# Gabriel-Ducrocq/GibbsSampler

Measured on AMD Instinct MI355X. Metric: Gibbs iters/sec (constrained-realization + C_l draw), Nside=512 lmax=1024, higher is better.
Workload: dtype f64

## Files before the change

gibbssampler_amd/_capi.py:

```python
import contextlib
import ctypes
import os

_HERE = os.path.dirname(os.path.abspath(__file__))
LIB_PATH = os.environ.get("GIBBS_HIP_LIB", os.path.join(_HERE, "libgibbs_hip.so"))

GS_MODE_CENTERED = 0
GS_MODE_NONCENTERED = 1
GS_QUIRK_ASIS_RECENTRE_CENTERED = 1
GS_NPARAM = 10
GS_ALM_REAL = 0
GS_ALM_COMPLEX = 1
GS_MCR_AUX, GS_MCR_OVERRELAX, GS_MCR_MALA, GS_MCR_AUX_MALA = 0, 1, 2, 3
NSTAT = {1: 2, 2: 4, 3: 8}

c_int_p = ctypes.POINTER(ctypes.c_int)
c_double_p = ctypes.POINTER(ctypes.c_double)


class GsModelDesc(ctypes.Structure):
    _fields_ = [
        ("lmax", ctypes.c_int),
        ("nside", ctypes.c_int),
        ("nfields", ctypes.c_int),
# ... 24 lines not shown
        ("mu_eps", ctypes.c_double),
        ("adj_iter", ctypes.c_int),
        ("nchains", ctypes.c_int),
        ("sht_mode", ctypes.c_int),
    ]


class GibbsHipError(RuntimeError):
    pass


_lib = None

_VP = ctypes.c_void_p
_SIGS = [
    ("gs_abi_version", ctypes.c_int, []),
    ("gs_last_error", ctypes.c_char_p, []),
    ("gs_option_set", ctypes.c_int, [ctypes.c_char_p, ctypes.c_char_p]),
    ("gs_option_get", ctypes.c_char_p, [ctypes.c_char_p]),
    ("gs_plan_create", ctypes.c_int, [ctypes.POINTER(GsModelDesc), ctypes.POINTER(_VP)]),
    ("gs_plan_destroy", ctypes.c_int, [_VP]),
    ("gs_plan_info", ctypes.c_int, [_VP, c_int_p, c_int_p, c_int_p, c_int_p]),
    ("gs_plan_sweep_info", ctypes.c_int, [_VP, c_int_p, c_int_p]),
    ("gs_var_expand", ctypes.c_int, [ctypes.c_int, ctypes.c_int, _VP, _VP, _VP]),
    ("gs_real_to_complex", ctypes.c_int, [ctypes.c_int, ctypes.c_int, _VP, _VP, _VP]),
    ("gs_complex_to_real", ctypes.c_int, [ctypes.c_int, ctypes.c_int, _VP, _VP, _VP]),
    ("gs_remove_monopole_dipole", ctypes.c_int, [ctypes.c_int, ctypes.c_int, _VP, _VP]),
    ("gs_alm2cl", ctypes.c_int, [ctypes.c_int, ctypes.c_int, _VP, _VP, _VP, _VP]),
    ("gs_unfold_bins", ctypes.c_int, [ctypes.c_int, _VP, _VP, ctypes.c_int, _VP, _VP]),
    ("gs_block_params", ctypes.c_int, [_VP, ctypes.c_int, _VP, _VP, _VP]),
    ("gs_cr_sweep", ctypes.c_int, [_VP, _VP, _VP, _VP, ctypes.c_uint64, ctypes.c_uint32, ctypes.c_uint32,
                                   _VP, _VP, _VP]),
    ("gs_sweep_stats", ctypes.c_int, [_VP, _VP, _VP, _VP, _VP]),
    ("gs_cls_draw", ctypes.c_int, [_VP, _VP, _VP, ctypes.c_uint64, ctypes.c_uint32, _VP, _VP]),
    ("gs_cls_scale_trace", ctypes.c_int, [_VP, _VP, ctypes.c_int, _VP]),
    ("gs_nc_mh", ctypes.c_int, [_VP, _VP, _VP, _VP, _VP, ctypes.c_uint64, ctypes.c_uint32, _VP, _VP]),
    ("gs_mh_adapt_enable", ctypes.c_int, [_VP, ctypes.c_double, ctypes.c_double]),
    ("gs_mh_adapt", ctypes.c_int, [_VP, _VP, _VP]),
    ("gs_mh_scale_get", ctypes.c_int, [_VP, _VP, _VP, _VP]),
    ("gs_mh_scale_set", ctypes.c_int, [_VP, _VP, _VP, _VP]),
    ("gs_mh_proposal_sd", ctypes.c_int, [_VP, _VP, _VP]),
    ("gs_stats_to_noncentered", ctypes.c_int, [_VP, _VP, _VP, _VP]),
    ("gs_recentre", ctypes.c_int, [_VP, _VP, _VP, _VP, _VP]),
    ("gs_step_centered", ctypes.c_int, [_VP, _VP, _VP, _VP, _VP, _VP, ctypes.c_uint64, ctypes.c_uint32, _VP]),
    ("gs_step_asis_fused", ctypes.c_int, [_VP, _VP, _VP, _VP, ctypes.c_uint64, ctypes.c_uint32, _VP, _VP, ctypes.c_int,
                                          _VP, ctypes.c_int, _VP]),
# ... 197 lines not shown
```

gibbssampler_amd/build.py:

```python
import glob
import os
import subprocess
import sys

HERE = os.path.dirname(os.path.abspath(__file__))
ROOT = os.path.dirname(HERE)
SOURCES = [os.path.join(HERE, "csrc", "gs_kernels.hip"), os.path.join(HERE, "csrc", "gs_sht.hip"),
           os.path.join(HERE, "csrc", "gs_masked.hip"), os.path.join(HERE, "csrc", "gs_summary.hip"),
           os.path.join(HERE, "csrc", "gs_br.hip")]
HEADERS = [os.path.join(HERE, "csrc", h) for h in ("gs_rng.h", "gs_common.h", "gs_bm_tables.h", "gs_block.h",
                                                         "gs_launch.h")] + \
    [os.path.join(ROOT, "include", "gibbs_capi.h")]
LIB = os.path.join(HERE, "libgibbs_hip.so")
ARCH = os.environ.get("GIBBS_OFFLOAD_ARCH", "gfx950")
COMMON = ["-ffp-contract=on"]
VARIANTS = {
    None: (LIB, ["-O3"] + COMMON),
    "debug": (os.path.join(HERE, "libgibbs_hip_debug.so"), ["-O3", "-DGS_DEBUG"] + COMMON),
    "timeline": (os.path.join(HERE, "libgibbs_hip_timeline.so"), ["-O3", "-DGS_MH_TIMELINE"] + COMMON),
    "asan": (os.path.join(HERE, "libgibbs_hip_asan.so"),
             ["-O1", "-g", "-fno-omit-frame-pointer", "-Xarch_host", "-fsanitize=address", "-shared-libasan"] + COMMON),
}


def asan_runtime():
    hits = sorted(glob.glob("/opt/rocm/lib/llvm/lib/clang/*/lib/linux/libclang_rt.asan-x86_64.so"))
    return hits[-1] if hits else None


def _stale(target, deps):
    if not os.path.exists(target):
        return True
    t = os.path.getmtime(target)
    return any(os.path.getmtime(d) > t for d in deps)
# ... 33 lines not shown
```

gibbssampler_amd/csrc/gs_kernels.hip:

```cpp
#include <hip/hip_runtime.h>
#include <stdint.h>
#include <math.h>
#include <string>
#include <vector>
#include <cstring>
#include <algorithm>
#include <cstdlib>
#include <map>
#include <mutex>

#include "gibbs_capi.h"
#include "gs_rng.h"
#include "gs_common.h"
#include "gs_block.h"
#include "gs_launch.h"

using namespace gs;

namespace {

using gs_detail::set_error;
using gs_detail::with_F;
using gs_detail::SeedWords;
using gs_detail::seed_words;
using gs_detail::nblk;

constexpr int WAVE = 64;
constexpr int NP = GS_NPARAM;
constexpr double PI = 3.14159265358979323846;

inline int nstat_of(int F) { return F == 1 ? GS_NSTAT_1 : (F == 2 ? GS_NSTAT_2 : GS_NSTAT_3); }
inline int nspec_of(int F) { return F == 1 ? 1 : (F == 2 ? 2 : 4); }

}

struct gs_plan {
    int device = 0;
    int L = 0, nside = 0, Npix = 0, F = 0, nchains = 0, chain0 = 0, quirks = 0, n_iter_mh = 1;
// ... 23 lines not shown
    int phase_sp[4][2] = {{-1, -1}, {-1, -1}, {-1, -1}, {-1, -1}};
    int* ell2blk = nullptr;
    double* gbuf = nullptr;
    double* bl = nullptr;
    int* ell2bin = nullptr;
    int* bins = nullptr;
    int* blocks = nullptr;
    double* prop_sd = nullptr;
    bool adapt_on = false;
    double adapt_target = 0.25, adapt_kappa = 0.6, adapt_lmax = 20.0;
    int nblk_mh = 0;
    std::vector<int> bin2blk_h;
    int* bin2blk = nullptr;
    double* mh_lam = nullptr;
    int* mh_cnt = nullptr;
    double* sd_chain = nullptr;
    int sd_stride = 0;
    const double* sd_tab() const { return adapt_on ? sd_chain : prop_sd; }
    int* meta = nullptr;
    int2* tasks = nullptr;
    int npair = 0, ntile = 0, nchunk = 0, rows_per_task = 64;
    int sweep_tw = 4, nchunkg = 0;
    int ntask = 0;
    double* partials = nullptr;
    bool raw_on = true;
    double* dmom = nullptr;
    const double* dmom_src = nullptr;
    double* params = nullptr;
    double* stats = nullptr;
    double* prop = nullptr;
    double* logr = nullptr;
    double* dl_tmp = nullptr;
    double* u_nat = nullptr;
    uint32_t* iter_dev = nullptr;
    bool cls_pre = false;
    bool cls_pre_many = false;
    double* cls_var = nullptr;
    double* scale_tr = nullptr;
    int scale_cap = 1;
    struct Deferred {
        bool pro_pending = false;
        const double* pro_dl = nullptr;
        gs_detail::SeedWords pro_seed{0, 0};
        uint32_t pro_it = 0;
        bool u_nat_ready = false;
        bool snap_ok = false;
// ... 407 lines not shown
    int n = 0;
    int nbp = 0, nbu = 0;
    int nspec = 0, nacc = 0, n_iter_mh = 0, maxbins = 0;
    const int* nbins = nullptr;
    const double* prop_sd = nullptr;
    int sd_stride = 0;
    const double* dl = nullptr;
    double* prop = nullptr;
    double* logr = nullptr;
    double* u_out = nullptr;
    double* snap = nullptr;
    int nbv = 0;
    ClsPre cp{};
};
template <int F>
__device__ void pro_pre_item(const ProPre& pp, int bx, int nchains, uint32_t seed_lo, uint32_t seed_hi, IterArg itarg,
                             int chain0);

#if defined(GS_SWEEP_WGTIME)
constexpr int SW_TL_MAX = 16384;
__device__ unsigned long long g_sw_tl[4 * SW_TL_MAX];
#endif

template <int F, int ZM, bool STORE, bool RAW = false>
__device__ __forceinline__ void cr_sweep_task(int wg, int L, int nchains, int ntile, int nchunkg, int tm, int tw,
                                              const int2* __restrict__ tasks, const double* __restrict__ d,
                                              const double* __restrict__ params, const double* __restrict__ z,
                                              double* __restrict__ s, double* __restrict__ partials,
                                              uint32_t seed_lo, uint32_t seed_hi, uint32_t iter, uint32_t substep,
                                              int chain0, const SweepOp& op, const double* __restrict__ tab,
                                              double* red) {
    constexpr int NS = SweepAcc<F>::n(RAW);
    const int pair = wg / nchains;
    const int chain = wg % nchains;
    const int lane = threadIdx.x & 63;
    const int2 gc = tasks[pair];
    if (gc.x < 0) return;
    const int w = threadIdx.x >> 6, cw = 4 / tw;
    const int t = tw * gc.x + w % tw;
    const bool tile_ok = t < ntile;
    const int lhi = L - WAVE * t;
    const int m0 = (cw * gc.y + w / tw) * tm;
    const int m1 = min(m0 + tm, lhi + 1);
    const bool active = tile_ok && m0 < m1;
    GS_ASSERT(gc.y < nchunkg && gc.x * tw < ntile);
    const int ell_lo = lhi - 63;
    const int ell = ell_lo + lane;
    const bool lane_ok = ell >= 0;
    const long long NR = (long long)(L + 1) * (L + 1);
    const Key key = chain_key(seed_lo, seed_hi, (uint32_t)(chain0 + chain));
    const uint32_t tag = TAG_CR | (substep << 8);

    double pm[NP];
    sweep_operator<F>(ZM != 2 && (!RAW || STORE) && lane_ok && active, chain, ell, L, params, op, pm);
    double acc[NS];
#pragma unroll
    for (int q = 0; q < NS; ++q) acc[q] = 0.0;

    const double* zc = ZM == 1 ? z + (long long)chain * F * NR : nullptr;
    double* sc = s + (long long)chain * F * NR;
// ... 43 lines not shown
                sweep_entry<F, ZM, STORE, 2, RAW>(dv, zc, sc, NR, (long long)r, i32, tag, iter, key, pm, acc, tab);
            }
            i32 += (uint32_t)(L - m);
        }
    } else {
        for (; m < m1; ++m) {
            if (lane_ok && ell >= m) {
                load_d<F, 2>(d, NR, 2 * i - (L + 1), dv);
                sweep_entry<F, ZM, STORE, 2, RAW>(dv, zc, sc, NR, 2 * i - (L + 1), (uint32_t)i, tag, iter, key, pm,
                                                 acc, tab);
            }
            i += L - m;
        }
    }
    double* po = partials + (((long long)chain * ntile + t) * nchunkg + gc.y) * NS * WAVE;
    sweep_partials_store<NS>(acc, tw, w, lane, tile_ok && (cw * gc.y) * tm <= lhi, po, red);
}

#ifndef GS_SWEEP_MINW
#define GS_SWEEP_MINW 1
#endif
template <int F, int ZM, bool STORE, int PRE = 0, bool RAW = false>
__global__ __launch_bounds__(256, GS_SWEEP_MINW) void k_cr_sweep(int L, int nchains, int ntile, int nchunkg, int tm, int tw,
                                                  const int2* __restrict__ tasks, const double* __restrict__ d,
                                                  const double* __restrict__ params, const double* __restrict__ z,
                                                  double* __restrict__ s, double* __restrict__ partials,
                                                  uint32_t seed_lo, uint32_t seed_hi, IterArg itarg, uint32_t substep,
                                                  int chain0, SweepOp op, ClsPre cp, ProPre pp, int nlog) {
    if constexpr (PRE == 0 && ZM == 0) {
        if ((int)blockIdx.x < pp.n) {
            pro_pre_item<F>(pp, (int)blockIdx.x, nchains, seed_lo, seed_hi, itarg, chain0);
            return;
        }
    }
    const uint32_t iter = itarg.get();
    constexpr int NS = SweepAcc<F>::n(RAW);
    __shared__ __attribute__((aligned(16))) double tab[ZM == 0 ? BM_TAB_DOUBLES : 2];
    __shared__ double red[3 * NS * WAVE];
    if constexpr (PRE > 0) {
        static_assert(ZM == 0, "latency form: native draws only");
        const int nsw = (int)gridDim.x - cp.n;
        if ((int)blockIdx.x >= nsw) {
            cls_variates_item<F>(cp, ((int)blockIdx.x - nsw) * blockDim.x + threadIdx.x, seed_lo, seed_hi, iter,
                                 chain0);
            return;
        }
        cr_sweep_latency<F, STORE, PRE, RAW>(L, nchains, ntile, nchunkg, tm, tw, tasks, d, s, partials, seed_lo,
                                        seed_hi, iter, substep, chain0, op, tab, red, (int)blockIdx.x, nsw);
        return;
    }
    if constexpr (ZM == 0) {
        bm_stage_tables(tab);
        __syncthreads();
    }
    const int bid = (int)blockIdx.x - pp.n;
    const int xcd = bid & 7, q8 = nlog >> 3, r8 = nlog & 7;
    const int base = xcd < r8 ? xcd * (q8 + 1) : r8 * (q8 + 1) + (xcd - r8) * q8;
#if defined(GS_SWEEP_WGTIME)
    const unsigned long long tl0 = wall_clock64();
#endif
    cr_sweep_task<F, ZM, STORE, RAW>(base + (bid >> 3), L, nchains, ntile, nchunkg, tm, tw, tasks, d, params, z, s,
                                partials, seed_lo, seed_hi, iter, substep, chain0, op, tab, red);
#if defined(GS_SWEEP_WGTIME)
    __syncthreads();
    if (threadIdx.x == 0 && bid < SW_TL_MAX) {
        unsigned long long* o = g_sw_tl + 4 * (size_t)bid;
        o[0] = tl0;
        o[1] = wall_clock64();
        o[2] = __builtin_amdgcn_s_getreg((31 << 11) | 4);
        o[3] = __builtin_amdgcn_s_getreg((31 << 11) | 20);
    }
#endif
}

template <int G>
__device__ __forceinline__ double stats_finish_sum(int L, int ntile, int nchunkg, int tm, int nstat,
                                                   const double* partials, int chain, int q, int t,
                                                   int w, int lane) {
    const int cmax = (L - WAVE * t) / tm;
    GS_ASSERT(cmax < nchunkg);
    const double* pp = partials + ((long long)chain * ntile + t) * nchunkg * nstat * WAVE + q * WAVE + lane;
    const long long cs = (long long)nstat * WAVE;
    double acc = 0.0;
    if constexpr (G <= 4) {
        int c = w;
// ... 1315 lines not shown
            const double r11 = An.a11 * t11;
            const double rB = An.aB * tB;
            for (int c = 0; c < nv; ++c) {
                const double sT = sc[0 * NR + r + c], sE = sc[1 * NR + r + c];
                sc[0 * NR + r + c] = r00 * sT;
                sc[1 * NR + r + c] = r10 * sT + r11 * sE;
                sc[2 * NR + r + c] *= rB;
            }
        }
    }
}

__global__ void k_iter_advance(uint32_t* it) { *it += 1u; }

__global__ void k_record_trace(long long n, const double* __restrict__ dl, double* __restrict__ trace, int capacity,
                               IterArg itarg) {
    const uint32_t it = itarg.get();
    const long long slot = (long long)((it + capacity - 1u) % (uint32_t)capacity);
    for (long long k = blockIdx.x * (long long)blockDim.x + threadIdx.x; k < n; k += (long long)gridDim.x * blockDim.x)
        trace[slot * n + k] = dl[k];
}

static const char* const k_options[] = {
    "GS_SWEEP_TW", "GS_SWEEP_THROUGHPUT", "GS_NC_RAW", "GS_NC_PIPE", "GS_MH_SPLIT", "GS_CLS_PRE", "GS_CLS_PRE_MANY", "GS_F2_GROUP_BYTES",
    "GS_F2_BATCH_BYTES", "GS_SHT_LDS_FFT_MAX", "GS_SHT_SEG", "GS_SHT_SYN", "GS_SHT_ANA", "GS_SHT_MERGE_RINGS",
    "GS_SHT_CONST_RINGS", "GS_SHT_BLOCKS_MFMA", "GS_SHT_BLK_STAGE", "GS_SHT_FUSED_AUX", "GS_SHT_MFMA_MAX_GB",
    "GS_SHT_RING_TW2"};
static bool opt_known(const char* name) {
    for (const char* k : k_options)
        if (std::strcmp(k, name) == 0) return true;
    return false;
}
static std::mutex& opt_mu() { static std::mutex m; return m; }
static std::map<std::string, std::string>& opt_tab() { static std::map<std::string, std::string> t; return t; }

const char* gs_detail::option(const char* name) {
    std::lock_guard<std::mutex> g(opt_mu());
    const auto it = opt_tab().find(name);
    return it == opt_tab().end() ? nullptr : it->second.c_str();
}

namespace {

template <typename T>
int dev_upload(T** dst, const std::vector<T>& src) {
    if (src.empty()) { *dst = nullptr; return 0; }
    GS_CHECK(hipMalloc((void**)dst, src.size() * sizeof(T)));
    GS_CHECK(hipMemcpy(*dst, src.data(), src.size() * sizeof(T), hipMemcpyHostToDevice));
    return 0;
}

template <typename T>
int dev_alloc(T** dst, size_t n) {
    GS_CHECK(hipMalloc((void**)dst, std::max<size_t>(n, 1) * sizeof(T)));
    GS_CHECK(hipMemset(*dst, 0, std::max<size_t>(n, 1) * sizeof(T)));
    return 0;
}

inline hipStream_t S(void* s) { return (hipStream_t)s; }

void build_tasks(gs_plan* p) {
    const int L = p->L;
    p->ntile = (L + 1 + WAVE - 1) / WAVE;
    auto waves = [&](int tm) {
        long long n = 0;
        for (int t = 0; t < p->ntile; ++t) n += (L - WAVE * t) / tm + 1;
        return n;
    };
    const int tm = L > 512 ? 16 : (L > 256 ? 4 : 8);
    p->rows_per_task = tm;
    p->nchunk = L / tm + 1;
    p->ntask = (int)waves(tm);
    int tw = 1;
    if (const char* env = gs_detail::option("GS_SWEEP_TW")) {
        const int v = atoi(env);
        if (v == 1 || v == 2 || v == 4) tw = v;
    }
    const int cw = 4 / tw;
    p->sweep_tw = tw;
    p->nchunkg = (p->nchunk + cw - 1) / cw;
    std::vector<std::pair<long long, int2>> work;
    for (int g = 0; tw * g < p->ntile; ++g)
        for (int c = 0; c * cw * tm <= L - WAVE * tw * g; ++c) {
            long long wl = 0;
            for (int t = tw * g; t < std::min(tw * g + tw, p->ntile); ++t) {
                const int lhi = L - WAVE * t, lo = std::max(lhi - 63, 0);
                for (int m = c * cw * tm; m < std::min((c + 1) * cw * tm, lhi + 1); ++m)
                    wl += lhi - std::max(lo, m) + 1;
            }
            work.push_back({wl, make_int2(g, c)});
        }
    std::stable_sort(work.begin(), work.end(), [](const auto& a, const auto& b) { return a.first > b.first; });
    const int per = (int)((work.size() + 7) / 8);
    std::vector<std::vector<int2>> bucket(8);
    std::vector<long long> load(8, 0);
    for (const auto& w : work) {
        int best = -1;
        for (int x = 0; x < 8; ++x)
            if ((int)bucket[x].size() < per && (best < 0 || load[x] < load[best])) best = x;
        bucket[best].push_back(w.second);
        load[best] += w.first;
    }
    std::vector<int2> tasks;
    for (int x = 0; x < 8; ++x) {
        for (const int2& t : bucket[x]) tasks.push_back(t);
        for (int k = (int)bucket[x].size(); k < per; ++k) tasks.push_back(make_int2(-1, 0));
    }
    p->npair = (int)tasks.size();
    dev_upload(&p->tasks, tasks);
}

int check_plan(const gs_plan* p) {
    if (!p) return set_error("null plan");
    return 0;
}

template <typename Fn>
void with_G(const gs_plan* p, Fn&& fn) {
    if (p->nchains <= 4) fn(std::integral_constant<int, 16>{});
    else fn(std::integral_constant<int, 4>{});
}

using SweepKernel = void (*)(int, int, int, int, int, int, const int2*, const double*, const double*, const double*,
                             double*, double*, uint32_t, uint32_t, IterArg, uint32_t, int, SweepOp, ClsPre, ProPre, int);

template <int F>
SweepKernel sweep_variant(bool lat, bool given, bool rep, bool raw, bool st) {
    if (lat && raw) return st ? k_cr_sweep<F, 0, true, 4, true> : k_cr_sweep<F, 0, false, 4, true>;
    if (lat) return st ? k_cr_sweep<F, 0, true, 4> : k_cr_sweep<F, 0, false, 4>;
    if (given) return k_cr_sweep<F, 2, false>;
    if (rep) return st ? k_cr_sweep<F, 1, true> : k_cr_sweep<F, 1, false>;
    if (raw) return st ? k_cr_sweep<F, 0, true, 0, true> : k_cr_sweep<F, 0, false, 0, true>;
    return st ? k_cr_sweep<F, 0, true> : k_cr_sweep<F, 0, false>;
}

}

extern "C" {

int gs_abi_version(void) { return GS_ABI_VERSION; }
const char* gs_last_error(void) { return gs_detail::g_last_error.c_str(); }

int gs_option_set(const char* name, const char* value) {
    if (!name || !opt_known(name)) return set_error(std::string("gs_option_set: unknown option ") + (name ? name : "(null)"));
    std::lock_guard<std::mutex> g(opt_mu());
    if (value) opt_tab()[name] = value; else opt_tab().erase(name);
// ... 174 lines not shown
    rc |= dev_alloc(&p->params, nc * (L + 1) * NP);
    rc |= dev_alloc(&p->stats, nc * p->nstat * (L + 1));
    rc |= dev_alloc(&p->prop, nc * p->nspec * maxbins);
    rc |= dev_alloc(&p->logr, nc * p->nspec * maxbins);
    rc |= dev_alloc(&p->dl_tmp, nc * p->nspec * maxbins);
    rc |= dev_alloc(&p->u_nat, nc * std::max(p->nacc, 1));
    rc |= dev_alloc(&p->iter_dev, 4);
    {
        const char* e = gs_detail::option("GS_CLS_PRE");
        p->cls_pre = e ? std::atoi(e) != 0 : p->nchains <= 4;
    }
    {
        const char* e = gs_detail::option("GS_CLS_PRE_MANY");
        p->cls_pre_many = !p->cls_pre && (e ? std::atoi(e) != 0 : true);
    }
    if (p->cls_pre || p->cls_pre_many) rc |= dev_alloc(&p->cls_var, nc * p->nspec * maxbins * 3);
    if (rc) { gs_plan_destroy(p); return -1; }
    *out = p;
    return 0;
}

int gs_plan_destroy(gs_plan* p) {
    if (!p) return 0;
    void* bufs[] = {p->iter_dev, p->ell2blk, p->gbuf, p->phase_tab, p->phase_rng, p->meta, p->bl, p->ell2bin, p->bins, p->blocks, p->prop_sd, p->tasks, p->partials, p->u_nat,
                    p->params, p->stats, p->prop, p->logr, p->dl_tmp, p->cls_var, p->phase_tab_s, p->phase_rng_s, p->dmom,
                    p->bin2blk, p->mh_lam, p->mh_cnt, p->sd_chain};
    for (void* b : bufs)
        if (b) (void)hipFree(b);
    if (p->pipe.slot[1]) (void)hipFree(p->pipe.slot[1]);
    for (hipEvent_t e : {p->pipe.ev_fork, p->pipe.ev_sweep[0], p->pipe.ev_sweep[1], p->pipe.ev_finish[0],
                         p->pipe.ev_finish[1]})
        if (e) (void)hipEventDestroy(e);
    if (p->pipe.side) (void)hipStreamDestroy(p->pipe.side);
    for (hipEvent_t e : p->ev) (void)hipEventDestroy(e);
    delete p;
    return 0;
}

int gs_plan_info(const gs_plan* p, int* maxbins, int* nstat, int* nblocks_total, int* nspec) {
    if (check_plan(p)) return -1;
    if (maxbins) *maxbins = p->maxbins;
    if (nstat) *nstat = p->nstat;
    if (nblocks_total) *nblocks_total = p->nacc;
    if (nspec) *nspec = p->nspec;
    return 0;
}

int gs_plan_sweep_info(const gs_plan* p, int* ntask, int* rows_per_task) {
    if (check_plan(p)) return -1;
    if (ntask) *ntask = p->ntask;
    if (rows_per_task) *rows_per_task = p->rows_per_task;
    return 0;
}

static int check_lmax_n(const char* fn, int lmax, int n, const void* a, const void* b) {
    if (lmax < 0 || n < 0) return set_error(std::string(fn) + ": lmax / n out of range");
    if (n > 0 && (!a || !b)) return set_error(std::string(fn) + ": null argument");
    return 0;
}

int gs_var_expand(int lmax, int n, const double* dl, double* var, void* stream) {
    if (check_lmax_n("gs_var_expand", lmax, n, dl, var)) return -1;
    if (n == 0) return 0;
    const long long nc = (long long)(lmax + 1) * (lmax + 2) / 2 * n;
    hipLaunchKernelGGL(k_var_expand, dim3(nblk(nc, 256)), dim3(256), 0, S(stream), lmax, n, dl, var);
    GS_LAUNCH_CHECK("k_var_expand");
    return 0;
}

int gs_real_to_complex(int lmax, int n, const double* re, double* cx, void* stream) {
    if (check_lmax_n("gs_real_to_complex", lmax, n, re, cx)) return -1;
    if (n == 0) return 0;
    const long long nc = (long long)(lmax + 1) * (lmax + 2) / 2 * n;
    hipLaunchKernelGGL(k_real_to_complex, dim3(nblk(nc, 256)), dim3(256), 0, S(stream), lmax, n, re, cx);
// ... 173 lines not shown
    bool raw = false;
    bool finish = true;
    SeedWords seed{0, 0};
    uint32_t iteration = 0, substep = 0;
    bool* cls_pre_done = nullptr;
    int slot = -1;
};

static int sweep_launch(gs_plan* p, const SweepReq& r, void* stream) {
    if (check_plan(p)) return -1;
    const bool raw_nost = r.raw && !r.s_out;
    if (!r.d_alm || !r.stats || (!r.given && !r.params && r.op_mode < 0 && !raw_nost) || (r.given && !r.s_out) ||
        ((r.op_mode >= 0 || r.raw) && !r.dl) || (r.raw && (r.given || r.z)))
        return set_error("gs_cr_sweep: null argument");
    const bool ahead = r.slot >= 0;
    if (ahead && (r.slot > 1 || !p->pipe.ready || !raw_nost || r.finish || r.cls_pre_done))
        return set_error("gs_cr_sweep: a sweep ahead is a raw-moment sweep alone, into a prepared slot");
    double* const partials = ahead ? p->pipe.slot[r.slot] : p->partials;
    if (!ahead) {
        p->defer.raw_pending = r.raw;
        p->defer.raw_dl = r.raw ? r.dl : nullptr;
    }
    const SweepOp op{r.op_mode, p->maxbins, r.dl, p->ell2bin, p->bl, p->kappa[0], p->kappa[1], p->kappa[2]};
    const int nlog = (int)((long long)p->nchains * p->npair);
    dim3 g((unsigned)nlog), b(256);
    hipEvent_t e0 = nullptr, e1 = nullptr;
    if (timing_begin(p, S(stream), &e0, &e1)) return -1;
    const bool rep = r.z != nullptr, st = r.s_out != nullptr;
    const bool lat = r.op_mode >= 0 && p->rows_per_task <= 4 && !r.given && !rep && p->sweep_latency;
    ClsPre cp{};
    ProPre pp{};
    if (r.cls_pre_done) *r.cls_pre_done = false;
    if (lat) {
        if (r.cls_pre_done && p->cls_pre) {
            cp = cls_front(p);
            g.x += cp.n;
            *r.cls_pre_done = true;
        }
    } else {
        if (!ahead && p->defer.pro_pending && !rep && !r.given && r.iteration == p->defer.pro_it) {
            pp = take_pro(p);
            p->defer.snap_ok = true;
        }
        if (r.cls_pre_done && p->cls_pre_many && !rep && !r.given && p->cls_var) {
            pp.cp = cls_front(p);
            pp.nbv = pp.cp.n;
            *r.cls_pre_done = true;
        }
        pp.n = (pp.nbp + pp.nbu + pp.nbv + 7) / 8 * 8;
        g.x += pp.n;
    }
    const SweepKernel k =
        with_F(p->F, [&](auto f) { return sweep_variant<decltype(f)::value>(lat, r.given, rep, r.raw, st); });
    hipLaunchKernelGGL(k, g, b, 0, S(stream), p->L, p->nchains, p->ntile, p->nchunkg, p->rows_per_task, p->sweep_tw,
                       p->tasks, r.d_alm, r.params, r.z, r.s_out, partials, r.seed.lo, r.seed.hi,
                       p->ita(r.iteration), r.substep, p->chain0, op, cp, pp, nlog);
    GS_LAUNCH_CHECK("k_cr_sweep");
    if (p->timing && record_ev(e1, S(stream))) return -1;
    return r.finish ? stats_finish(p, r.stats, stream) : 0;
}

int gs_cr_sweep(gs_plan* p, const double* d_alm, const double* params, const double* z, uint64_t seed,
                uint32_t iteration, uint32_t substep, double* s_out, double* stats, void* stream) {
    SweepReq r;
    r.d_alm = d_alm; r.params = params; r.z = z; r.s_out = s_out; r.stats = stats;
    r.seed = seed_words(seed); r.iteration = iteration; r.substep = substep;
    return sweep_launch(p, r, stream);
}

int gs_sweep_stats(gs_plan* p, const double* d_alm, const double* s, double* stats, void* stream) {
    SweepReq r;
    r.d_alm = d_alm; r.s_out = const_cast<double*>(s); r.stats = stats; r.given = true;
    return sweep_launch(p, r, stream);
}

static int cls_draw_launch(gs_plan* p, const double* stats, const double* variates, uint64_t seed,
                           uint32_t iteration, double* dl_out, double* trace, int cap, uint32_t* counter,
                           void* stream, const double* pre = nullptr) {
// ... 669 lines not shown
```

gibbssampler_amd/engine.py:

```python
import ctypes
import math

import numpy as np
import torch
from scipy.stats import invgamma

from . import _capi as C

SPECTRA = {1: ("TT",), 2: ("EE", "BB"), 3: ("TT", "EE", "BB", "TE")}
FIELDS = {1: ("TT",), 2: ("EE", "BB"), 3: ("TT", "EE", "BB")}
MH_ORDER = {1: ("TT",), 2: ("EE", "BB"), 3: ("EE", "BB", "TT", "TE")}


def _require_gpu():
    if not torch.cuda.is_available():
        raise C.GibbsHipError("gibbssampler_amd needs a ROCm GPU (MI355X); no CPU fallback")


class GibbsPlan:
    def __init__(self, lmax, nside, nfields, nchains, bl, noise_var, bins, blocks=None,
                 proposal_variances=None, chain0=0, quirks=C.GS_QUIRK_ASIS_RECENTRE_CENTERED,
                 n_iter_metropolis=1, device=None):
        _require_gpu()
        self.lib = C.load()
# ... 29 lines not shown
            desc.nbin_edges[k] = len(b)
            if self.blocks is not None:
                bk = np.ascontiguousarray(self.blocks[s], dtype=np.int32)
                keep.append(bk)
                desc.blocks[k] = bk.ctypes.data_as(C.c_int_p)
                desc.nblock_edges[k] = len(bk)
            if self.proposal_variances is not None:
                pv = np.ascontiguousarray(self.proposal_variances[s], dtype=np.float64)
                if len(pv) != len(b) - 1 - 2:
                    raise ValueError(f"proposal_variances[{s}] must have nbins-2 entries")
                keep.append(pv)
                desc.prop_var[k] = pv.ctypes.data_as(C.c_double_p)
        h = ctypes.c_void_p()
        with torch.cuda.device(self.device):
            C.check(self.lib.gs_plan_create(ctypes.byref(desc), ctypes.byref(h)), "gs_plan_create")
        self._h = h
        mb, ns, nacc, nsp = (ctypes.c_int() for _ in range(4))
        C.check(self.lib.gs_plan_info(h, ctypes.byref(mb), ctypes.byref(ns), ctypes.byref(nacc), ctypes.byref(nsp)))
        self.maxbins, self.nstat, self.nacc, self.nspec = mb.value, ns.value, nacc.value, nsp.value
        self.NR = (self.L + 1) ** 2
        nt, rpt = ctypes.c_int(), ctypes.c_int()
        C.check(self.lib.gs_plan_sweep_info(h, ctypes.byref(nt), ctypes.byref(rpt)))
        self.ntask, self.rows_per_task = nt.value, rpt.value
        ell = np.arange(self.L + 1, dtype=np.float64)
        expo = (2 * ell + 1) / 2
        self._alphas = {}
        for s in self.spectra:
            b = self.bins[s]
            a = np.array([np.sum(expo[b[i]:b[i + 1]]) - 1 for i in range(len(b) - 1)])
            a[0] = 1
            self._alphas[s] = a
        self.adapting = False
        self.scale_trace = None
        self._acc_layout = []
        if self.blocks is not None:
            for s in MH_ORDER[self.F]:
                self._acc_layout.append((s, (len(self.blocks[s]) - 1) * self.n_iter_metropolis))

    def __del__(self):
        try:
            C.park(dict(self.__dict__))
            if getattr(self, "_h", None) is not None and self.lib is not None:
                C.release(self.lib.gs_plan_destroy, self._h)
                self._h = None
        except Exception:
            pass
# ... 382 lines not shown
```

include/gibbs_capi.h:

```cpp
#ifndef GIBBS_CAPI_H
#define GIBBS_CAPI_H

#include <stdint.h>

#ifdef __cplusplus
extern "C" {
#endif

#define GS_ABI_VERSION 1

#define GS_MODE_CENTERED 0
#define GS_MODE_NONCENTERED 1

#define GS_QUIRK_ASIS_RECENTRE_CENTERED 1

#define GS_NSTAT_1 2
#define GS_NSTAT_2 4
#define GS_NSTAT_3 8
#define GS_NPARAM 10

typedef struct gs_plan gs_plan;

typedef struct gs_model_desc {
    int lmax;
// ... 2 lines not shown
    int nchains;
    int chain0;
    int quirks;
    int n_iter_metropolis;
    const double* bl;
    const double* noise_var;
    const int* bins[4];
    int nbin_edges[4];
    const int* blocks[4];
    int nblock_edges[4];
    const double* prop_var[4];
} gs_model_desc;

int gs_abi_version(void);
const char* gs_last_error(void);

int gs_option_set(const char* name, const char* value);
const char* gs_option_get(const char* name);

int gs_plan_create(const gs_model_desc* desc, gs_plan** out);
int gs_plan_destroy(gs_plan* plan);
int gs_plan_info(const gs_plan* plan, int* maxbins, int* nstat, int* nblocks_total, int* nspec);
int gs_plan_sweep_info(const gs_plan* plan, int* ntask, int* rows_per_task);

int gs_var_expand(int lmax, int n, const double* dl, double* var, void* stream);
int gs_real_to_complex(int lmax, int n, const double* re, double* cplx_interleaved, void* stream);
int gs_complex_to_real(int lmax, int n, const double* cplx_interleaved, double* re, void* stream);
int gs_remove_monopole_dipole(int lmax, int n, double* alm, void* stream);
int gs_alm2cl(int lmax, int n, const double* x, const double* y, double* cl, void* stream);
int gs_unfold_bins(int n, const double* binned, const int* bins, int nbins, double* out, void* stream);

int gs_block_params(gs_plan* plan, int mode, const double* dl_binned, double* params, void* stream);
int gs_cr_sweep(gs_plan* plan, const double* d_alm, const double* params, const double* z_replay,
                uint64_t seed, uint32_t iteration, uint32_t substep,
                double* s_out, double* stats, void* stream);
int gs_sweep_stats(gs_plan* plan, const double* d_alm, const double* s, double* stats, void* stream);
int gs_cls_draw(gs_plan* plan, const double* stats, const double* invgamma_replay,
                uint64_t seed, uint32_t iteration, double* dl_binned_out, void* stream);
int gs_cls_scale_trace(gs_plan* plan, double* scales, int capacity, void* stream);
int gs_mh_propose(gs_plan* plan, const double* dl, const double* u_prop, uint64_t seed, uint32_t iteration,
                  double* prop_out, double* logr_out, double* u_acc_out, void* stream);
int gs_nc_mh(gs_plan* plan, const double* stats, double* dl_binned,
             const double* u_prop_replay, const double* u_accept_replay,
             uint64_t seed, uint32_t iteration, int32_t* accept_out, void* stream);
int gs_mh_adapt_enable(gs_plan* plan, double target, double kappa);
int gs_mh_adapt(gs_plan* plan, const int32_t* accept, void* stream);
// ... 138 lines not shown
```

Measured before the change: 199,800.

## Pack ragged triangular sweep chunks so waves carry balanced row counts

Adds a host-built packing plan that re-sorts the 256 (tile, chunk, lane) segments of each chunk group by row count, so each wave's loop trip count matches its longest member instead of idling on the triangular edge. Optionally absorbs a trailing single-row chunk into the preceding group. Packed groups are dispatched through a separate task list with a per-thread decoded word table and a four-plane LDS reduction. It runs only for the non-latency, non-replay, non-store sweep path when tw==1, and adds table loads and a more complex reduction.

```diff
diff --git a/gibbssampler_amd/_capi.py b/gibbssampler_amd/_capi.py
--- a/gibbssampler_amd/_capi.py
+++ b/gibbssampler_amd/_capi.py
@@ -70,6 +70,7 @@
     ("gs_plan_destroy", ctypes.c_int, [_VP]),
     ("gs_plan_info", ctypes.c_int, [_VP, c_int_p, c_int_p, c_int_p, c_int_p]),
     ("gs_plan_sweep_info", ctypes.c_int, [_VP, c_int_p, c_int_p]),
+    ("gs_plan_sweep_pack_info", ctypes.c_int, [_VP, c_int_p, c_int_p]),
     ("gs_var_expand", ctypes.c_int, [ctypes.c_int, ctypes.c_int, _VP, _VP, _VP]),
     ("gs_real_to_complex", ctypes.c_int, [ctypes.c_int, ctypes.c_int, _VP, _VP, _VP]),
     ("gs_complex_to_real", ctypes.c_int, [ctypes.c_int, ctypes.c_int, _VP, _VP, _VP]),
diff --git a/gibbssampler_amd/build.py b/gibbssampler_amd/build.py
--- a/gibbssampler_amd/build.py
+++ b/gibbssampler_amd/build.py
@@ -9,7 +9,7 @@
            os.path.join(HERE, "csrc", "gs_masked.hip"), os.path.join(HERE, "csrc", "gs_summary.hip"),
            os.path.join(HERE, "csrc", "gs_br.hip")]
 HEADERS = [os.path.join(HERE, "csrc", h) for h in ("gs_rng.h", "gs_common.h", "gs_bm_tables.h", "gs_block.h",
-                                                         "gs_launch.h")] + \
+                                                         "gs_launch.h", "gs_sweep_pack.h")] + \
     [os.path.join(ROOT, "include", "gibbs_capi.h")]
 LIB = os.path.join(HERE, "libgibbs_hip.so")
 ARCH = os.environ.get("GIBBS_OFFLOAD_ARCH", "gfx950")
diff --git a/gibbssampler_amd/csrc/gs_kernels.hip b/gibbssampler_amd/csrc/gs_kernels.hip
--- a/gibbssampler_amd/csrc/gs_kernels.hip
+++ b/gibbssampler_amd/csrc/gs_kernels.hip
@@ -14,6 +14,7 @@
 #include "gs_common.h"
 #include "gs_block.h"
 #include "gs_launch.h"
+#include "gs_sweep_pack.h"
 
 using namespace gs;
 
@@ -83,6 +84,10 @@
     int npair = 0, ntile = 0, nchunk = 0, rows_per_task = 64;
     int sweep_tw = 4, nchunkg = 0;
     int ntask = 0;
+    int2* tasks_pk = nullptr;
+    int npair_pk = 0;
+    int npacked = 0, nabsorb = 0;
+    int* pack_tab = nullptr;
     double* partials = nullptr;
     bool raw_on = true;
     double* dmom = nullptr;
@@ -536,9 +541,78 @@
 __device__ unsigned long long g_sw_tl[4 * SW_TL_MAX];
 #endif
 
-template <int F, int ZM, bool STORE, bool RAW = false>
+template <int F, bool RAW, int NPLANE>
+__device__ __forceinline__ void cr_sweep_packed(int chain, int4 pd, const int* __restrict__ pack, int L, int ntile,
+                                                int nchunkg, int tm, const double* __restrict__ d,
+                                                const double* __restrict__ params, double* __restrict__ partials,
+                                                uint32_t seed_lo, uint32_t seed_hi, uint32_t iter, uint32_t substep,
+                                                int chain0, const SweepOp& op, const double* __restrict__ tab,
+                                                double* red) {
+    static_assert(NPLANE == 4, "the packed form sums four chunk planes of `red`");
+    constexpr int NS = SweepAcc<F>::n(RAW);
+    const int t = pd.x, cg = pd.y;
+    const gs_pack::Word wd = gs_pack::decode((uint32_t)pack[pd.z + (int)threadIdx.x]);
+    const int trips = __builtin_amdgcn_readfirstlane(wd.trips);
+    const int lhi = L - WAVE * t;
+    const int ell = wd.single ? lhi : lhi - 63 + wd.lt;
+    int m = (wd.single ? 4 * cg + 4 : 4 * cg + wd.cq) * tm;
+    int cnt = wd.cnt;
+    GS_ASSERT(t < ntile && cg + (pd.w ? 1 : 0) < nchunkg && (cnt == 0 || (ell >= 0 && m + cnt - 1 <= ell)));
+    const long long NR = (long long)(L + 1) * (L + 1);
+    const Key key = chain_key(seed_lo, seed_hi, (uint32_t)(chain0 + chain));
+    const uint32_t tag = TAG_CR | (substep << 8);
+    double pm[NP];
+    sweep_operator<F>(!RAW && cnt > 0, chain, max(ell, 0), L, params, op, pm);
+    double acc[NS];
+#pragma unroll
+    for (int q = 0; q < NS; ++q) acc[q] = 0.0;
+    double dv[F][2];
+    if (cnt > 0 && m == 0) {
+        load_d<F, 1>(d, NR, ell, dv);
+        sweep_entry<F, 0, false, 1, RAW>(dv, nullptr, nullptr, NR, ell, (uint32_t)ell, tag, iter, key, pm, acc, tab);
+        m = 1;
+        --cnt;
+    }
+    const char* db[F];
+#pragma unroll
+    for (int f = 0; f < F; ++f) db[f] = reinterpret_cast<const char*>(d + (size_t)f * (size_t)NR);
+    GS_ASSERT(NR * 8 < (1ll << 32));
+    uint32_t i32 = (uint32_t)((long long)m * (2 * L + 1 - m) / 2 + ell);
+    for (int j = 0; j < trips; ++j) {
+        if (j < cnt) {
+            const uint32_t r = 2u * i32 - (uint32_t)(L + 1);
+            GS_ASSERT((long long)r + 1 < NR && (long long)r > L);
+            load_d2_off<F>(db, r * 8u, dv);
+            sweep_entry<F, 0, false, 2, RAW>(dv, nullptr, nullptr, NR, (long long)r, i32, tag, iter, key, pm, acc, tab);
+        }
+        i32 += (uint32_t)(L - m);
+        ++m;
+    }
+    double* po = partials + (((long long)chain * ntile + t) * nchunkg + cg) * NS * WAVE;
+#pragma unroll
+    for (int q = 0; q < NS; ++q) red[(wd.cq * NS + q) * WAVE + wd.lt] = wd.single ? 0.0 : acc[q];
+    if (wd.single)
+#pragma unroll
+        for (int q = 0; q < NS; ++q) po[(NS + q) * WAVE + 63] = acc[q];
+    __syncthreads();
+    const int w = threadIdx.x >> 6, lane = threadIdx.x & 63;
+    if (w == 0) {
+#pragma unroll
+        for (int q = 0; q < NS; ++q) {
+            double v = red[q * WAVE + lane];
+            for (int k = 1; k < 4; ++k) v += red[(k * NS + q) * WAVE + lane];
+            po[q * WAVE + lane] = v;
+        }
+    } else if (w == 1 && pd.w && lane < 63) {
+#pragma unroll
+        for (int q = 0; q < NS; ++q) po[(NS + q) * WAVE + lane] = 0.0;
+    }
+}
+
+template <int F, int ZM, bool STORE, bool RAW = false, int NPLANE = 3>
 __device__ __forceinline__ void cr_sweep_task(int wg, int L, int nchains, int ntile, int nchunkg, int tm, int tw,
-                                              const int2* __restrict__ tasks, const double* __restrict__ d,
+                                              const int2* __restrict__ tasks, const int* __restrict__ pack,
+                                              const double* __restrict__ d,
                                               const double* __restrict__ params, const double* __restrict__ z,
                                               double* __restrict__ s, double* __restrict__ partials,
                                               uint32_t seed_lo, uint32_t seed_hi, uint32_t iter, uint32_t substep,
@@ -549,7 +623,14 @@
     const int chain = wg % nchains;
     const int lane = threadIdx.x & 63;
     const int2 gc = tasks[pair];
-    if (gc.x < 0) return;
+    if (gc.x < 0) {
+        if constexpr (ZM == 0 && !STORE && NPLANE == 4) {
+            if (gc.x < -1)
+                cr_sweep_packed<F, RAW, NPLANE>(chain, reinterpret_cast<const int4*>(pack)[-2 - gc.x], pack, L, ntile, nchunkg,
+                                        tm, d, params, partials, seed_lo, seed_hi, iter, substep, chain0, op, tab, red);
+        }
+        return;
+    }
     const int w = threadIdx.x >> 6, cw = 4 / tw;
     const int t = tw * gc.x + w % tw;
     const bool tile_ok = t < ntile;
@@ -639,7 +720,8 @@
 #endif
 template <int F, int ZM, bool STORE, int PRE = 0, bool RAW = false>
 __global__ __launch_bounds__(256, GS_SWEEP_MINW) void k_cr_sweep(int L, int nchains, int ntile, int nchunkg, int tm, int tw,
-                                                  const int2* __restrict__ tasks, const double* __restrict__ d,
+                                                  const int2* __restrict__ tasks, const int* __restrict__ pack,
+                                                  const double* __restrict__ d,
                                                   const double* __restrict__ params, const double* __restrict__ z,
                                                   double* __restrict__ s, double* __restrict__ partials,
                                                   uint32_t seed_lo, uint32_t seed_hi, IterArg itarg, uint32_t substep,
@@ -653,7 +735,8 @@
     const uint32_t iter = itarg.get();
     constexpr int NS = SweepAcc<F>::n(RAW);
     __shared__ __attribute__((aligned(16))) double tab[ZM == 0 ? BM_TAB_DOUBLES : 2];
-    __shared__ double red[3 * NS * WAVE];
+    constexpr int NPLANE = ZM == 0 && !STORE && PRE == 0 ? 4 : 3;
+    __shared__ double red[NPLANE * NS * WAVE];
     if constexpr (PRE > 0) {
         static_assert(ZM == 0, "latency form: native draws only");
         const int nsw = (int)gridDim.x - cp.n;
@@ -676,8 +759,9 @@
 #if defined(GS_SWEEP_WGTIME)
     const unsigned long long tl0 = wall_clock64();
 #endif
-    cr_sweep_task<F, ZM, STORE, RAW>(base + (bid >> 3), L, nchains, ntile, nchunkg, tm, tw, tasks, d, params, z, s,
-                                partials, seed_lo, seed_hi, iter, substep, chain0, op, tab, red);
+    cr_sweep_task<F, ZM, STORE, RAW, NPLANE>(base + (bid >> 3), L, nchains, ntile, nchunkg, tm, tw, tasks, pack, d,
+                                             params, z, s, partials, seed_lo, seed_hi, iter, substep, chain0, op, tab,
+                                             red);
 #if defined(GS_SWEEP_WGTIME)
     __syncthreads();
     if (threadIdx.x == 0 && bid < SW_TL_MAX) {
@@ -2039,7 +2123,7 @@
 }
 
 static const char* const k_options[] = {
-    "GS_SWEEP_TW", "GS_SWEEP_THROUGHPUT", "GS_NC_RAW", "GS_NC_PIPE", "GS_MH_SPLIT", "GS_CLS_PRE", "GS_CLS_PRE_MANY", "GS_F2_GROUP_BYTES",
+    "GS_SWEEP_TW", "GS_SWEEP_PACK", "GS_SWEEP_THROUGHPUT", "GS_NC_RAW", "GS_NC_PIPE", "GS_MH_SPLIT", "GS_CLS_PRE", "GS_CLS_PRE_MANY", "GS_F2_GROUP_BYTES",
     "GS_F2_BATCH_BYTES", "GS_SHT_LDS_FFT_MAX", "GS_SHT_SEG", "GS_SHT_SYN", "GS_SHT_ANA", "GS_SHT_MERGE_RINGS",
     "GS_SHT_CONST_RINGS", "GS_SHT_BLOCKS_MFMA", "GS_SHT_BLK_STAGE", "GS_SHT_FUSED_AUX", "GS_SHT_MFMA_MAX_GB",
     "GS_SHT_RING_TW2"};
@@ -2084,7 +2168,7 @@
         for (int t = 0; t < p->ntile; ++t) n += (L - WAVE * t) / tm + 1;
         return n;
     };
-    const int tm = L > 512 ? 16 : (L > 256 ? 4 : 8);
+    const int tm = gs_pack::rows_per_chunk(L);
     p->rows_per_task = tm;
     p->nchunk = L / tm + 1;
     p->ntask = (int)waves(tm);
@@ -2107,24 +2191,53 @@
             }
             work.push_back({wl, make_int2(g, c)});
         }
-    std::stable_sort(work.begin(), work.end(), [](const auto& a, const auto& b) { return a.first > b.first; });
-    const int per = (int)((work.size() + 7) / 8);
-    std::vector<std::vector<int2>> bucket(8);
-    std::vector<long long> load(8, 0);
-    for (const auto& w : work) {
-        int best = -1;
-        for (int x = 0; x < 8; ++x)
-            if ((int)bucket[x].size() < per && (best < 0 || load[x] < load[best])) best = x;
-        bucket[best].push_back(w.second);
-        load[best] += w.first;
-    }
-    std::vector<int2> tasks;
-    for (int x = 0; x < 8; ++x) {
-        for (const int2& t : bucket[x]) tasks.push_back(t);
-        for (int k = (int)bucket[x].size(); k < per; ++k) tasks.push_back(make_int2(-1, 0));
-    }
+    auto deal = [](std::vector<std::pair<long long, int2>>& work) {
+        std::stable_sort(work.begin(), work.end(), [](const auto& a, const auto& b) { return a.first > b.first; });
+        const int per = (int)((work.size() + 7) / 8);
+        std::vector<std::vector<int2>> bucket(8);
+        std::vector<long long> load(8, 0);
+        for (const auto& w : work) {
+            int best = -1;
+            for (int x = 0; x < 8; ++x)
+                if ((int)bucket[x].size() < per && (best < 0 || load[x] < load[best])) best = x;
+            bucket[best].push_back(w.second);
+            load[best] += w.first;
+        }
+        std::vector<int2> tasks;
+        for (int x = 0; x < 8; ++x) {
+            for (const int2& t : bucket[x]) tasks.push_back(t);
+            for (int k = (int)bucket[x].size(); k < per; ++k) tasks.push_back(make_int2(-1, 0));
+        }
+        return tasks;
+    };
+    const std::vector<int2> tasks = deal(work);
     p->npair = (int)tasks.size();
     dev_upload(&p->tasks, tasks);
+    const char* pk = gs_detail::option("GS_SWEEP_PACK");
+    if (tw != 1 || (pk && atoi(pk) == 0)) return;
+    const gs_pack::Plan P = gs_pack::build(L, tm, true);
+    std::map<std::pair<int, int>, long long> plain_wl;
+    for (const auto& w : work) plain_wl[{w.second.x, w.second.y}] = w.first;
+    std::vector<std::pair<long long, int2>> work_pk;
+    std::vector<int> tab;
+    for (const gs_pack::Group& g : P.groups)
+        if (g.packed) {
+            work_pk.push_back({(long long)WAVE * g.rows_issued, make_int2(-2 - (int)tab.size() / 4, 0)});
+            const int desc[4] = {g.tile, g.cg, g.cls, g.absorb ? 1 : 0};
+            ++p->npacked;
+            p->nabsorb += g.absorb ? 1 : 0;
+            tab.insert(tab.end(), desc, desc + 4);
+        } else {
+            work_pk.push_back({plain_wl.at({g.tile, g.cg}), make_int2(g.tile, g.cg)});
+        }
+    if (tab.empty()) return;
+    const int nd = (int)tab.size();
+    for (int k = 0; k < nd; k += 4) tab[k + 2] = nd + tab[k + 2] * gs_pack::NTHREAD;
+    tab.insert(tab.end(), P.table.begin(), P.table.end());
+    const std::vector<int2> tasks_pk = deal(work_pk);
+    p->npair_pk = (int)tasks_pk.size();
+    dev_upload(&p->tasks_pk, tasks_pk);
+    dev_upload(&p->pack_tab, tab);
 }
 
 int check_plan(const gs_plan* p) {
@@ -2138,7 +2251,7 @@
     else fn(std::integral_constant<int, 4>{});
 }
 
-using SweepKernel = void (*)(int, int, int, int, int, int, const int2*, const double*, const double*, const double*,
+using SweepKernel = void (*)(int, int, int, int, int, int, const int2*, const int*, const double*, const double*, const double*,
                              double*, double*, uint32_t, uint32_t, IterArg, uint32_t, int, SweepOp, ClsPre, ProPre, int);
 
 template <int F>
@@ -2359,7 +2472,7 @@
 
 int gs_plan_destroy(gs_plan* p) {
     if (!p) return 0;
-    void* bufs[] = {p->iter_dev, p->ell2blk, p->gbuf, p->phase_tab, p->phase_rng, p->meta, p->bl, p->ell2bin, p->bins, p->blocks, p->prop_sd, p->tasks, p->partials, p->u_nat,
+    void* bufs[] = {p->iter_dev, p->ell2blk, p->gbuf, p->phase_tab, p->phase_rng, p->meta, p->bl, p->ell2bin, p->bins, p->blocks, p->prop_sd, p->tasks, p->tasks_pk, p->pack_tab, p->partials, p->u_nat,
                     p->params, p->stats, p->prop, p->logr, p->dl_tmp, p->cls_var, p->phase_tab_s, p->phase_rng_s, p->dmom,
                     p->bin2blk, p->mh_lam, p->mh_cnt, p->sd_chain};
     for (void* b : bufs)
@@ -2387,6 +2500,13 @@
     if (check_plan(p)) return -1;
     if (ntask) *ntask = p->ntask;
     if (rows_per_task) *rows_per_task = p->rows_per_task;
+    return 0;
+}
+
+int gs_plan_sweep_pack_info(const gs_plan* p, int* npacked, int* nabsorbed) {
+    if (check_plan(p)) return -1;
+    if (npacked) *npacked = p->tasks_pk ? p->npacked : 0;
+    if (nabsorbed) *nabsorbed = p->tasks_pk ? p->nabsorb : 0;
     return 0;
 }
 
@@ -2606,12 +2726,14 @@
         p->defer.raw_dl = r.raw ? r.dl : nullptr;
     }
     const SweepOp op{r.op_mode, p->maxbins, r.dl, p->ell2bin, p->bl, p->kappa[0], p->kappa[1], p->kappa[2]};
-    const int nlog = (int)((long long)p->nchains * p->npair);
+    const bool rep = r.z != nullptr, st = r.s_out != nullptr;
+    const bool lat = r.op_mode >= 0 && p->rows_per_task <= 4 && !r.given && !rep && p->sweep_latency;
+    const bool packed = p->tasks_pk && !lat && !r.given && !rep && !st;
+    const int2* const tasks = packed ? p->tasks_pk : p->tasks;
+    const int nlog = (int)((long long)p->nchains * (packed ? p->npair_pk : p->npair));
     dim3 g((unsigned)nlog), b(256);
     hipEvent_t e0 = nullptr, e1 = nullptr;
     if (timing_begin(p, S(stream), &e0, &e1)) return -1;
-    const bool rep = r.z != nullptr, st = r.s_out != nullptr;
-    const bool lat = r.op_mode >= 0 && p->rows_per_task <= 4 && !r.given && !rep && p->sweep_latency;
     ClsPre cp{};
     ProPre pp{};
     if (r.cls_pre_done) *r.cls_pre_done = false;
@@ -2637,7 +2759,7 @@
     const SweepKernel k =
         with_F(p->F, [&](auto f) { return sweep_variant<decltype(f)::value>(lat, r.given, rep, r.raw, st); });
     hipLaunchKernelGGL(k, g, b, 0, S(stream), p->L, p->nchains, p->ntile, p->nchunkg, p->rows_per_task, p->sweep_tw,
-                       p->tasks, r.d_alm, r.params, r.z, r.s_out, partials, r.seed.lo, r.seed.hi,
+                       tasks, p->pack_tab, r.d_alm, r.params, r.z, r.s_out, partials, r.seed.lo, r.seed.hi,
                        p->ita(r.iteration), r.substep, p->chain0, op, cp, pp, nlog);
     GS_LAUNCH_CHECK("k_cr_sweep");
     if (p->timing && record_ev(e1, S(stream))) return -1;
diff --git a/gibbssampler_amd/csrc/gs_sweep_pack.h b/gibbssampler_amd/csrc/gs_sweep_pack.h
--- /dev/null
+++ b/gibbssampler_amd/csrc/gs_sweep_pack.h
@@ -0,0 +1,133 @@
+#pragma once
+#include <algorithm>
+#include <cstdint>
+#include <map>
+#include <vector>
+
+#if defined(__HIPCC__)
+#define GS_PACK_HD __host__ __device__
+#else
+#define GS_PACK_HD
+#endif
+
+namespace gs_pack {
+
+constexpr int TILE = 64;
+constexpr int CPG = 4;
+constexpr int NTHREAD = TILE * CPG;
+
+inline int rows_per_chunk(int L) { return L > 512 ? 16 : (L > 256 ? 4 : 8); }
+
+struct Word {
+    int lt, cq, cnt, trips;
+    bool single;
+};
+GS_PACK_HD inline uint32_t encode(const Word& w) {
+    return (uint32_t)w.lt | (uint32_t)w.cq << 6 | (uint32_t)w.cnt << 8 | (uint32_t)w.trips << 13 |
+           (uint32_t)(w.single ? 1 : 0) << 18;
+}
+GS_PACK_HD inline Word decode(uint32_t u) {
+    return Word{(int)(u & 63u), (int)(u >> 6 & 3u), (int)(u >> 8 & 31u), (int)(u >> 13 & 31u), (u >> 18 & 1u) != 0};
+}
+
+inline int seg_rows(int L, int tm, int tile, int cg, int cq, int lt) {
+    const int l = L - TILE * tile - (TILE - 1) + lt;
+    const int m0 = (CPG * cg + cq) * tm;
+    return l < m0 ? 0 : std::min(tm, l - m0 + 1);
+}
+
+struct Group {
+    int tile = 0, cg = 0;
+    bool packed = false;
+    bool absorb = false;
+    int cls = -1;
+    int rows_plain = 0;
+    int rows_issued = 0;
+};
+
+struct Plan {
+    int L = 0, tm = 0, ntile = 0, nchunkg = 0;
+    std::vector<Group> groups;
+    std::vector<uint32_t> table;
+    int ncls = 0;
+    long long rows_plain = 0, rows_issued = 0;
+};
+
+inline int pack_group(int L, int tm, int tile, int cg, bool absorb, uint32_t (&out)[NTHREAD]) {
+    Word w[NTHREAD];
+    for (int cq = 0; cq < CPG; ++cq)
+        for (int lt = 0; lt < TILE; ++lt)
+            w[cq * TILE + lt] = Word{lt, cq, seg_rows(L, tm, tile, cg, cq, lt), 0, false};
+    std::stable_sort(w, w + NTHREAD, [](const Word& a, const Word& b) { return a.cnt > b.cnt; });
+    if (absorb) {
+        int k = 0;
+        while (k < NTHREAD && w[k].cnt > 0) ++k;
+        if (k == NTHREAD) return -1;
+        w[k].cnt = 1;
+        w[k].single = true;
+    }
+    int issued = 0;
+    for (int v = 0; v < CPG; ++v) {
+        int trips = 0, pre = 0;
+        for (int k = v * TILE; k < (v + 1) * TILE; ++k) {
+            const int first0 = (!w[k].single && cg == 0 && w[k].cq == 0 && w[k].cnt > 0) ? 1 : 0;
+            trips = std::max(trips, w[k].cnt - first0);
+            pre = std::max(pre, first0);
+        }
+        for (int k = v * TILE; k < (v + 1) * TILE; ++k) w[k].trips = trips;
+        issued += trips + pre;
+    }
+    for (int k = 0; k < NTHREAD; ++k) out[k] = encode(w[k]);
+    return issued;
+}
+
+inline Plan build(int L, int tm, bool pack) {
+    Plan P;
+    P.L = L;
+    P.tm = tm;
+    P.ntile = (L + TILE) / TILE;
+    P.nchunkg = (L / tm + 1 + CPG - 1) / CPG;
+    std::map<std::vector<uint32_t>, int> classes;
+    for (int t = 0; t < P.ntile; ++t) {
+        const int lhi = L - TILE * t;
+        for (int c = 0; c * CPG * tm <= lhi; ++c) {
+            Group g;
+            g.tile = t;
+            g.cg = c;
+            for (int cq = 0; cq < CPG; ++cq) {
+                const int m0 = (CPG * c + cq) * tm;
+                g.rows_plain += std::max(0, std::min(m0 + tm, lhi + 1) - m0);
+            }
+            g.rows_issued = g.rows_plain;
+            P.rows_plain += g.rows_plain;
+            if (pack) {
+                const bool single_next = lhi == CPG * (c + 1) * tm;
+                uint32_t words[NTHREAD];
+                int issued = pack_group(L, tm, t, c, single_next, words);
+                bool absorb = single_next && issued >= 0;
+                if (single_next && !absorb) issued = pack_group(L, tm, t, c, false, words);
+                if (absorb || issued < g.rows_plain) {
+                    g.packed = true;
+                    g.absorb = absorb;
+                    g.rows_issued = issued;
+                    const std::vector<uint32_t> key(words, words + NTHREAD);
+                    auto it = classes.find(key);
+                    if (it == classes.end()) {
+                        it = classes.emplace(key, P.ncls++).first;
+                        P.table.insert(P.table.end(), key.begin(), key.end());
+                    }
+                    g.cls = it->second;
+                }
+            }
+            P.rows_issued += g.rows_issued;
+            P.groups.push_back(g);
+            if (g.absorb) {
+                P.rows_plain += 1;
+                ++c;
+            }
+        }
+    }
+    return P;
+}
+
+}
diff --git a/gibbssampler_amd/engine.py b/gibbssampler_amd/engine.py
--- a/gibbssampler_amd/engine.py
+++ b/gibbssampler_amd/engine.py
@@ -75,6 +75,8 @@
         nt, rpt = ctypes.c_int(), ctypes.c_int()
         C.check(self.lib.gs_plan_sweep_info(h, ctypes.byref(nt), ctypes.byref(rpt)))
         self.ntask, self.rows_per_task = nt.value, rpt.value
+        C.check(self.lib.gs_plan_sweep_pack_info(h, ctypes.byref(nt), ctypes.byref(rpt)))
+        self.sweep_packed, self.sweep_absorbed = nt.value, rpt.value
         ell = np.arange(self.L + 1, dtype=np.float64)
         expo = (2 * ell + 1) / 2
         self._alphas = {}
diff --git a/include/gibbs_capi.h b/include/gibbs_capi.h
--- a/include/gibbs_capi.h
+++ b/include/gibbs_capi.h
@@ -48,6 +48,7 @@
 int gs_plan_destroy(gs_plan* plan);
 int gs_plan_info(const gs_plan* plan, int* maxbins, int* nstat, int* nblocks_total, int* nspec);
 int gs_plan_sweep_info(const gs_plan* plan, int* ntask, int* rows_per_task);
+int gs_plan_sweep_pack_info(const gs_plan* plan, int* npacked, int* nabsorbed);
 
 int gs_var_expand(int lmax, int n, const double* dl, double* var, void* stream);
 int gs_real_to_complex(int lmax, int n, const double* re, double* cplx_interleaved, void* stream);
```

Measured after the change: 201,900 (median of 6 runs). +1.0%, better.
